# arpg/Kangaroo

Measured on AMD Instinct MI355X. Metric: kinectfusion_frames_per_sec_640x480_to_512cubed_tsdf, higher is better.
Workload: dtype f32

## Files before the change

include/kfx_debug.h:

```cpp
#ifndef KFX_DEBUG_H
#define KFX_DEBUG_H

#include "kfx.h"

#ifdef __cplusplus
extern "C" {
#endif

int kfx_debug_rmw(const kfx_volume* vol, int variant, kfx_stream stream);

int kfx_debug_div_uniform_check(float b, unsigned long long* d_out, kfx_stream stream);

int kfx_debug_div_core_check(unsigned seed, int per_divisor, unsigned long long* d_out, kfx_stream stream);
int kfx_debug_sqrt_core_check(unsigned long long* d_out, kfx_stream stream);
int kfx_debug_wave_xor_check(unsigned seed, unsigned long long* d_out, kfx_stream stream);

int kfx_debug_summary_export(kfx_sdf_summary* s, float tol, float vref, int fine_shift, void* R_out, void* C_out, int dims_out[12],
                             kfx_stream stream);


#ifdef __cplusplus
}
#endif
#endif
```

kangaroo_amd/csrc/debug.hip:

```cpp
#include "kfx_device.h"
#include "sampling.h"
#include "../../include/kfx_debug.h"

namespace kfx {

__global__ __launch_bounds__(256) void k_rmw_linear(float4* __restrict__ base, size_t n4)
{
    const size_t stride = (size_t)gridDim.x * blockDim.x;
    for (size_t i = (size_t)blockIdx.x * blockDim.x + threadIdx.x; i < n4; i += stride) {
        float4 c = base[i];
        c.y += 1.0f;
        c.w += 1.0f;
        base[i] = c;
    }
}

template <int ZC>
__global__ __launch_bounds__(256) void k_rmw_brick(unsigned char* vptr, size_t pitch, size_t img_pitch, int X, int Y, int Z)
{
    const int tid = threadIdx.x, lane = tid & 63, wv = tid >> 6;
    const int x0 = (blockIdx.x * 32 + (lane & 31)) * 2;
    const int y = blockIdx.y * 8 + wv * 2 + (lane >> 5);
    const int zbeg = blockIdx.z * ZC, zend = min(zbeg + ZC, Z);
    if (x0 >= X || y >= Y) return;
// ... 221 lines not shown
    default: return set_error(KFX_E_RANGE, "kfx_debug_rmw: variant");
    }
    return check_launch("kfx_debug_rmw");
}

extern "C" int kfx_debug_summary_export(kfx_sdf_summary* s, float tol, float vref, int fine_shift, void* R_out, void* C_out, int dims_out[12],
                                        kfx_stream stream)
{
    if (!s || !dims_out) return set_error(KFX_E_NULL, "kfx_debug_summary_export: null argument");
    if (fine_shift < 3 || fine_shift > 5) return set_error(KFX_E_RANGE, "kfx_debug_summary_export: fine_shift in [3, 5]");
    ClassView cv;
    summary_class_layout(s, fine_shift, cv);
    dims_out[0] = s->nbx; dims_out[1] = s->nby; dims_out[2] = s->nbz;
    dims_out[3] = cv.fine.first; dims_out[4] = cv.fine.rw; dims_out[5] = cv.fine.ny;
    dims_out[6] = cv.coarse.first; dims_out[7] = cv.coarse.rw; dims_out[8] = cv.coarse.ny;
    dims_out[9] = cv.words; dims_out[10] = s->n_coarse; dims_out[11] = (s->h_skippable && s->builds) ? ((volatile int*)s->h_skippable)[(s->builds - 1) % KFX_SUMMARY_RING] : -2;
    const size_t n = (size_t)s->nbx * s->nby * s->nbz;
    hipStream_t st = (hipStream_t)stream;
    if (R_out && hipMemcpyAsync(R_out, s->R, n * sizeof(float4), hipMemcpyDeviceToDevice, st) != hipSuccess) return set_error(KFX_E_RANGE, "kfx_debug_summary_export: copy");
    if (C_out) {
        if (int e = summary_classes_prepare(s, tol, vref, fine_shift, st)) return e;
        if (hipMemcpyAsync(C_out, s->C, (size_t)cv.words * sizeof(unsigned), hipMemcpyDeviceToDevice, st) != hipSuccess || hipStreamSynchronize(st) != hipSuccess)
            return set_error(KFX_E_RANGE, "kfx_debug_summary_export: copy");
        dims_out[11] = (s->h_skippable && s->builds) ? ((volatile int*)s->h_skippable)[(s->builds - 1) % KFX_SUMMARY_RING] : -2;
    }
    return 0;
}
```

kangaroo_amd/csrc/frame.hip:

```cpp
#include <cmath>
#include <cstdlib>
#include <new>

#include "kfx_device.h"

struct kfx_frame {
    kfx_frame_config cfg;
    kfx_sdf_summary* summary;
    int track;
    long long frames;
    int slots;
    hipEvent_t* ev;
    long long* ev_frame;
    unsigned char* ev_mask;
    unsigned mask;
    kfx_image texels;
};

using namespace kfx;

static int valid_image(const kfx_image& im, size_t elem)
{
    return im.ptr && im.w > 0 && im.h > 0 && im.pitch >= im.w * elem;
}
// ... 135 lines not shown
        f->ev_frame[(int)(f->frames % f->slots)] = -1;
    }
    const hipStream_t s = (hipStream_t)stream;
    int e = 0;
    const auto record = [&](int k) {
        if (!(m & (1u << k))) return;
        const hipError_t he = hipEventRecord(ev[k], s);
        if (he != hipSuccess) {
            (void)hipGetLastError();
            f->ev_mask[(int)(f->frames % f->slots)] &= (unsigned char)~(1u << k);
            if (!e) e = set_error((int)he, "kfx_frame_step: hipEventRecord");
        }
    };
    record(0);
    const kfx_image* tex = ((parts & KFX_FRAME_PREPROCESS) && (parts & KFX_FRAME_FUSE) && f->texels.ptr) ? &f->texels : nullptr;
    if (!e && (parts & KFX_FRAME_PREPROCESS)) {
        e = kfx_bilateral_f32(&c.filtered, src, c.bilateral_gs, c.bilateral_gr, c.bilateral_size, c.bilateral_minval, 1, stream);
        if (!e) e = depth_to_vbo_normals_texels(&c.vbo, &c.normals, &c.filtered, c.K, 1.0f, tex, stream);
    }
    record(1);
    if (!e && (parts & KFX_FRAME_FUSE))
        e = sdf_fuse_texels(&c.vol, f->track ? f->summary : nullptr, &c.filtered, &c.normals, tex, T_cw, c.K, c.trunc_dist, c.max_w, c.mincostheta, c.fuse_flags, stream);
    record(2);
    if (!e && (parts & KFX_FRAME_RAYCAST)) {
        if (f->track) e = kfx_raycast_sdf_tracked(&c.ray_depth, &c.ray_norm, &c.ray_img, &c.vol, f->summary, T_wc, c.K, c.near, c.far, c.trunc_dist, 1, stream);
        else e = kfx_raycast_sdf(&c.ray_depth, &c.ray_norm, &c.ray_img, &c.vol, T_wc, c.K, c.near, c.far, c.trunc_dist, 1, stream);
    }
    record(3);
    f->frames += 1;
    return e;
}

extern "C" int kfx_frame_timings(kfx_frame* f, long long first_frame, int n_frames, float* ms)
{
// ... 50 lines not shown
```

kangaroo_amd/csrc/kfx_device.h:

```cpp
#pragma once

#include <hip/hip_runtime.h>
#include <stddef.h>
#include <stdint.h>

#include "../../include/kfx.h"
#include "../../include/kfx_extras.h"

namespace kfx {

struct V3 { float x, y, z; };

__device__ __forceinline__ V3 v3(float x, float y, float z) { return V3{x, y, z}; }
__device__ __forceinline__ V3 operator+(V3 a, V3 b) { return V3{a.x + b.x, a.y + b.y, a.z + b.z}; }
__device__ __forceinline__ V3 operator-(V3 a, V3 b) { return V3{a.x - b.x, a.y - b.y, a.z - b.z}; }
__device__ __forceinline__ V3 operator*(V3 a, float s) { return V3{a.x * s, a.y * s, a.z * s}; }
__device__ __forceinline__ V3 div_cw(V3 a, V3 b) { return V3{a.x / b.x, a.y / b.y, a.z / b.z}; }
__device__ __forceinline__ V3 div_s(V3 a, float s) { const float inv = 1.0f / s; return a * inv; }
__device__ __forceinline__ float dot(V3 a, V3 b) { return a.x * b.x + a.y * b.y + a.z * b.z; }
__device__ __forceinline__ float length(V3 a) { return sqrtf(dot(a, a)); }
__device__ __forceinline__ float lerp(float a, float b, float t) { return a + t * (b - a); }
__device__ __forceinline__ V3 lerp(V3 a, V3 b, float t) { return a + (b - a) * t; }
__device__ __forceinline__ float clampf(float f, float a, float b) { return fmaxf(a, fminf(f, b)); }

// ... 111 lines not shown
}

#define KFX_SUMMARY_RING 8
struct kfx_sdf_summary {
    float4* R;
    int nbx, nby, nbz;
    int w, h, d;
    const unsigned char* base;
    size_t pitch, img_pitch;
    unsigned* C;
    int c_dirty;
    float c_tol, c_vref;
    int c_shift;
    int n_coarse;
    int* d_count;
    int* h_skippable;
    int* d_skippable;
    hipEvent_t build_done[8];
    unsigned builds;
    unsigned plain_calls;
    unsigned sweeps;
};
namespace kfx {
struct ClassLevel {
    int shift;
    int ny;
    int rw;
    int first;
};
struct ClassView {
    const unsigned* C;
    ClassLevel fine, coarse;
    int words;
    float vref;
    float tol;
    int amb_ok;
    int ox, oy, oz;
    float eps;
    int nx5, nz5, top_n, lds_words;
};
inline __host__ __device__ void class_level_up(const int nx, const int ny, const int nz, const int shift, const int first, ClassLevel& L, int& ux, int& uz, int& words)
{
    ux = (nx + 1) >> 1; uz = (nz + 1) >> 1;
    L.shift = shift; L.ny = (ny + 1) >> 1; L.rw = 2 * ((ux + 31) >> 5); L.first = first;
    words = (L.rw * L.ny * uz + 3) & ~3;
}
int summary_classes_prepare(kfx_sdf_summary* s, float tol, float vref, int fine_shift, hipStream_t stream);
void summary_class_layout(const kfx_sdf_summary* s, int fine_shift, ClassView& cv);
int summary_view_offset(const kfx_sdf_summary* s, const kfx_volume* view, int* ox, int* oy, int* oz);
}

namespace kfx {
int set_error(int code, const char* what);
int check_launch(const char* what);
int math_mode();
size_t texel_image_bytes(size_t w, size_t h);
int depth_to_vbo_normals_texels(const kfx_image* vbo, const kfx_image* nrm, const kfx_image* depth, const float K[4], float scale,
                                const kfx_image* texels, kfx_stream stream);
int sdf_fuse_slab_texels(const kfx_volume* vol, const kfx_slab* slab, const kfx_image* depth, const kfx_image* norm, const kfx_image* texels,
                         const float T_cw[12], const float K[4], float trunc_dist, float max_w, float mincostheta, unsigned flags, kfx_stream stream);
int sdf_fuse_texels(const kfx_volume* vol, kfx_sdf_summary* summary, const kfx_image* depth, const kfx_image* norm, const kfx_image* texels,
                    const float T_cw[12], const float K[4], float trunc_dist, float max_w, float mincostheta, unsigned flags, kfx_stream stream);
}
```

kangaroo_amd/csrc/preprocess.hip:

```cpp
#include <cstdlib>

#include "kfx_device.h"

namespace kfx {

constexpr int BIL_MAX_R = 16;

struct BilParams {
    const unsigned char* in;
    size_t in_pitch;
    unsigned char* out;
    size_t out_pitch;
    int w, h;
    int iw, ih;
    int R;
    float gs, gr;
    float minval;
    int use_minval;
};

template <typename Ti>
__device__ __forceinline__ float load_clamped(const BilParams& p, int x, int y)
{
    x = min(max(x, 0), p.iw - 1);
// ... 44 lines not shown
                    if (!p.use_minval || q >= p.minval) {
                        const float id = pc - q;
                        const float id2 = id * id;
                        const float iw = __expf(-(id2) / inv2gr);
                        const float w = srow[c] * iw;
                        sumw += w;
                        sum += w * q;
                    }
                }
            }
        }
        reinterpret_cast<float*>(p.out + (size_t)y * p.out_pitch)[x] = sum / sumw;
    }
}

template <typename Ti, int R>
__global__ __launch_bounds__(256) void k_bilateral_fast(const BilParams p)
{
    constexpr int TX = 16, TY = 16, D = 2 * R + 1, TW = TX + 2 * R, TH = TY + 2 * R;
    __shared__ float tile[TH * TW];
    __shared__ float sw[D * D];
    const int tid = threadIdx.x;
    const int bx = blockIdx.x * TX, by = blockIdx.y * TY;
    for (int i = tid; i < TW * TH; i += 256) {
        const int ty = i / TW, tx = i - ty * TW;
        tile[i] = load_clamped<Ti>(p, bx + tx - R, by + ty - R);
    }
    if (tid < D * D) {
        const int r = tid / D - R, c = tid % D - R;
        sw[tid] = __expf(-((float)(r * r + c * c)) / (2 * p.gs * p.gs));
    }
    __syncthreads();
    const int lx = tid % TX, ly = tid / TX;
    const int x = bx + lx, y = by + ly;
    if (x >= p.w || y >= p.h) return;
    const float k = -1.0f / (2 * p.gr * p.gr);
    const float pc = tile[(ly + R) * TW + lx + R];
    const bool check = p.use_minval != 0;
    float sum = 0.f, sumw = 0.f;
#pragma unroll
    for (int r = 0; r < D; ++r)
#pragma unroll
        for (int c = 0; c < D; ++c) {
            const float q = tile[(ly + r) * TW + lx + c];
            const bool ok = !check || q >= p.minval;
            const float id = pc - q;
            const float w = sw[r * D + c] * __expf(id * id * k);
            sumw += ok ? w : 0.f;
            sum += ok ? w * q : 0.f;
        }
    if (check && !(pc >= p.minval)) sum = sumw = 0.f;
    reinterpret_cast<float*>(p.out + (size_t)y * p.out_pitch)[x] = sum / sumw;
}

template <typename Ti>
__global__ __launch_bounds__(256) void k_bilateral_global(const BilParams p)
{
    const int x = blockIdx.x * 64 + (threadIdx.x & 63), y = blockIdx.y * 4 + (threadIdx.x >> 6);
    if (x >= p.w || y >= p.h) return;
    const float pc = (float)reinterpret_cast<const Ti*>(p.in + (size_t)y * p.in_pitch)[x];
    float sum = 0.f, sumw = 0.f;
    if (!p.use_minval || pc >= p.minval) {
        for (int r = -p.R; r <= p.R; ++r)
            for (int c = -p.R; c <= p.R; ++c) {
                const float q = load_clamped<Ti>(p, x + c, y + r);
                if (!p.use_minval || q >= p.minval) {
                    const float sd2 = (float)(r * r + c * c);
// ... 89 lines not shown
}

struct VboNrmParams {
    const unsigned char* in;
    size_t in_pitch;
    unsigned char *vbo, *nrm;
    size_t vpitch, npitch;
    int w, h;
    Intr K;
    float scale;
    unsigned char* tex;
    size_t tpitch;
    float* bmax;
    unsigned bw8;
};
__device__ __forceinline__ float4 vertex_of(const VboNrmParams& p, int u, int v)
{
    const float kz = p.scale * reinterpret_cast<const float*>(p.in + (size_t)v * p.in_pitch)[u];
    return make_float4(kz * ((float)u - p.K.u0) / p.K.fu, kz * ((float)v - p.K.v0) / p.K.fv, kz, 1.0f);
}
__global__ __launch_bounds__(256) void k_vbo_normals_f32(const VboNrmParams p)
{
    __shared__ float s_max[4][8];
    const int lane = threadIdx.x & 63, wv = threadIdx.x >> 6;
    const int u = blockIdx.x * 64 + lane, v = blockIdx.y * 4 + wv;
    float d = -__builtin_inff();
    if (u < p.w && v < p.h) {
        const float4 Vc = vertex_of(p, u, v);
        reinterpret_cast<float4*>(p.vbo + (size_t)v * p.vpitch)[u] = Vc;
        float4 N = make_float4(0.f, 0.f, 0.f, 0.f);
        if (u + 1 < p.w && v + 1 < p.h) {
            const float4 Vr = vertex_of(p, u + 1, v), Vu = vertex_of(p, u, v + 1);
            const V3 a = v3(Vr.x - Vc.x, Vr.y - Vc.y, Vr.z - Vc.z);
            const V3 b = v3(Vu.x - Vc.x, Vu.y - Vc.y, Vu.z - Vc.z);
            const V3 axb = v3(a.y * b.z - a.z * b.y, a.z * b.x - a.x * b.z, a.x * b.y - a.y * b.x);
            const float mag = length(axb);
            N = make_float4(-axb.x / mag, -axb.y / mag, -axb.z / mag, 1.0f);
        }
        reinterpret_cast<float4*>(p.nrm + (size_t)v * p.npitch)[u] = N;
        if (p.tex) {
            d = reinterpret_cast<const float*>(p.in + (size_t)v * p.in_pitch)[u];
            reinterpret_cast<float4*>(p.tex + (size_t)v * p.tpitch)[u] = make_float4(N.x, N.y, N.z, d);
        }
    }
    if (p.tex) {
        d = wave8_combine(fmaxf(d, -__builtin_inff()), [](float a, float b) { return fmaxf(a, b); });
        if ((lane & 7) == 0) s_max[wv][lane >> 3] = d;
        __syncthreads();
        if (threadIdx.x < 8)
            p.bmax[(size_t)blockIdx.y * p.bw8 + blockIdx.x * 8 + threadIdx.x] =
                fmaxf(fmaxf(s_max[0][threadIdx.x], s_max[1][threadIdx.x]), fmaxf(s_max[2][threadIdx.x], s_max[3][threadIdx.x]));
    }
}

struct EwParams {
    const unsigned char* in;
    size_t in_pitch;
    unsigned char* out;
    size_t out_pitch;
    int w, h;
    float s, offset;
};

__global__ __launch_bounds__(256) void k_scale_bias_f32(const EwParams p)
{
    const int x = blockIdx.x * 64 + (threadIdx.x & 63), y = blockIdx.y * 4 + (threadIdx.x >> 6);
// ... 407 lines not shown
    if (int e = check_image(depth, 4, "DepthToVbo+Normals: depth image")) return e;
    if (!K) return set_error(KFX_E_NULL, "DepthToVbo+Normals: null intrinsics");
    if (vbo->w == 0 || vbo->h == 0) return 0;
    if (nrm->w != vbo->w || nrm->h != vbo->h || depth->w < vbo->w || depth->h < vbo->h)
        return set_error(KFX_E_SHAPE, "DepthToVbo+Normals: image sizes");
    const size_t tpitch = (vbo->w * 16 + 255) / 256 * 256;
    if (texels && (!texels->ptr || texels->w != vbo->w || texels->h != vbo->h || texels->pitch != tpitch || ((uintptr_t)texels->ptr & 15)))
        return set_error(KFX_E_SHAPE, "DepthToVbo+Normals: texel image");
    VboNrmParams p{(const unsigned char*)depth->ptr, depth->pitch, (unsigned char*)vbo->ptr, (unsigned char*)nrm->ptr, vbo->pitch, nrm->pitch,
                   (int)vbo->w, (int)vbo->h, Intr{K[0], K[1], K[2], K[3]}, scale, texels ? (unsigned char*)texels->ptr : nullptr, texels ? tpitch : 0,
                   texels ? reinterpret_cast<float*>((unsigned char*)texels->ptr + tpitch * vbo->h) : nullptr, (unsigned)((vbo->w + 63) / 64 * 8)};
    hipLaunchKernelGGL(k_vbo_normals_f32, dim3(ceil_div(p.w, 64), ceil_div(p.h, 4)), dim3(256), 0, (hipStream_t)stream, p);
    return check_launch("kfx_depth_to_vbo_normals_f32");
}

struct PyrParams {
    const unsigned char* d0;
    size_t d0_pitch;
    unsigned char* d[4];
    size_t dpitch[4];
    unsigned char *vbo[4], *nrm[4];
    size_t vpitch[4], npitch[4];
    int w[4], h[4];
    Intr K[4];
    int levels;
    float scale;
};
__device__ __forceinline__ float4 pyr_vertex(const Intr& K, float scale, float depth, int u, int v)
{
    const float kz = scale * depth;
// ... 139 lines not shown
```

kangaroo_amd/csrc/raycast.hip:

```cpp
#include <cmath>
#include <cstdlib>

#include <hip/hip_fp16.h>

#include "kfx_device.h"
#include "sampling.h"

namespace kfx {

struct RayParams {
    VolView vol;
    V3 size;
    V3 dims1;
    V3 hi2;
    V3 voxel;
    V3 inv_size;
    int fastdiv, off32;
    Pose T;
    Intr K;
    unsigned char *dptr, *nptr, *iptr;
    size_t dpitch, npitch, ipitch;
    int w, h;
    float near, far, trunc;
    int subpix;
// ... 737 lines not shown
    static const int kb_env = [] { const char* e = getenv("KFX_RAYCAST_CLASS_KB"); const int v = e ? atoi(e) : 16; return v < 1 ? 1 : (v > 60 ? 60 : v); }();
    int fine = 3;
    for (; fine < 5; ++fine) {
        summary_class_layout(summary, fine, cl);
        if ((size_t)cl.words * 4 <= (size_t)kb_env * 1024) break;
    }
    summary_class_layout(summary, fine, cl);
    if ((size_t)cl.words * 4 > 60 * 1024) return 0;
    const float tol = math_mode() == KFX_MATH_FAST ? 1e-5f : 0.f;
    static const int force_env = [] { const char* e = getenv("KFX_RAYCAST_SUMMARY"); return e ? atoi(e) : 0; }();
    if (force_env < 0) return 0;
    const bool steer = force_env == 0 && summary->h_skippable;
    if (steer && summary->plain_calls && (summary->plain_calls++ % 8u) != 0u) return 0;
    if (int e = summary_classes_prepare(summary, tol, p.trunc, fine, (hipStream_t)stream)) return e;
    if (steer && summary->builds >= 3) {
        const unsigned ref = (summary->builds - 3) % KFX_SUMMARY_RING;
        (void)hipEventSynchronize(summary->build_done[ref]);
        const int known = ((volatile int*)summary->h_skippable)[ref];
        if (known >= 0 && (long long)known * 4 < summary->n_coarse) {
            if (!summary->plain_calls) summary->plain_calls = 1;
            return 0;
        }
        summary->plain_calls = 0;
    }
    cl.C = summary->C;
    cl.vref = p.trunc;
    cl.amb_ok = p.trunc >= p.voxel.x ? 1 : 0;
    cl.tol = tol;
    const double u24 = 1.0 / 16777216.0;
    double eps = 0.0;
    const float bmin[3] = {p.vol.bmin.x, p.vol.bmin.y, p.vol.bmin.z}, bmax[3] = {p.vol.bmax.x, p.vol.bmax.y, p.vol.bmax.z};
    const float size[3] = {p.size.x, p.size.y, p.size.z}, dims1[3] = {p.dims1.x, p.dims1.y, p.dims1.z};
    const float cw[3] = {p.T.m[3], p.T.m[7], p.T.m[11]};
// ... 336 lines not shown
```

kangaroo_amd/csrc/summary.hip:

```cpp
#include <algorithm>
#include <new>

#include "kfx_device.h"

namespace kfx {

__global__ __launch_bounds__(256) void k_summary_fill(float4* __restrict__ R, size_t n, float lo, float hi, int state)
{
    const size_t i = (size_t)blockIdx.x * 256 + threadIdx.x;
    if (i < n) R[i] = make_float4(lo, hi, __int_as_float(state), 0.f);
}

struct ClassBuild {
    const float4* R;
    unsigned* C;
    int nbx, nby, nbz;
    int shift, nx, ny, nz, rw;
    float lo_ok, hi_ok;
    const unsigned* src;
    int src_shift, src_nx, src_ny, src_nz, src_rw;
};
template <int M>
__device__ __forceinline__ int class_row(const ClassBuild& b, const long long wave)
{
    const float4* __restrict__ R = b.R;
    unsigned* __restrict__ C = b.C;
    const unsigned* __restrict__ src = b.src;
    const int nbx = b.nbx, nby = b.nby, nbz = b.nbz, shift = b.shift, nx = b.nx, ny = b.ny, rw = b.rw;
    const int src_shift = b.src_shift, src_nx = b.src_nx, src_ny = b.src_ny, src_nz = b.src_nz, src_rw = b.src_rw;
    const float lo_ok = b.lo_ok, hi_ok = b.hi_ok;
    const int lane = threadIdx.x & 63;
    const int chunks = (nx + 63) >> 6;
    const int chunk = (int)(wave % chunks), by = (int)((wave / chunks) % ny), bz = (int)(wave / ((long long)chunks * ny));
    const int bx = chunk * 64 + lane;
    int cls = 0;
    if (bx < nx) {
        bool all_nan = true, all_free = true, all_either = true;
        if constexpr (M == 0) {
            const int m = 1 << (shift - src_shift);
            for (int z0 = 0; z0 < m; z0 += 2) {
                uint2 w2[2][4];
#pragma unroll
                for (int dz = 0; dz < 2; ++dz)
#pragma unroll
                    for (int dy = 0; dy < 4; ++dy) {
                        const int z = min(bz * m + z0 + dz, src_nz - 1), y = min(by * m + min(dy, m - 1), src_ny - 1);
                        w2[dz][dy] = *reinterpret_cast<const uint2*>(src + ((size_t)z * src_ny + y) * src_rw + (((bx * m) >> 5) << 1));
                    }
// ... 29 lines not shown
#pragma unroll
                    for (int dx = 0; dx <= M; ++dx)
                        r[(dz * (M + 1) + dy) * (M + 1) + dx] =
                            R[((size_t)min(bz * M + dz, nbz - 1) * nby + min(by * M + dy, nby - 1)) * nbx + min(bx * M + dx, nbx - 1)];
#pragma unroll
            for (int k = 0; k < (M + 1) * (M + 1) * (M + 1); ++k) {
                const int st = __float_as_int(r[k].z);
                const bool in_band = r[k].x >= lo_ok && r[k].y <= hi_ok;
                all_nan = all_nan && st == 1;
                all_free = all_free && st == 0 && in_band;
                all_either = all_either && (st == 1 || in_band);
            }
        }
        cls = all_free ? 1 : (all_nan ? 2 : (all_either ? 3 : 0));
    }
    const unsigned long long p0 = __ballot(cls & 1), p1 = __ballot(cls & 2);
    if (lane == 0) {
        unsigned* row = C + ((size_t)bz * ny + by) * rw + chunk * 4;
        row[0] = (unsigned)p0; row[1] = (unsigned)p1;
        if (chunk * 4 + 2 < rw) { row[2] = (unsigned)(p0 >> 32); row[3] = (unsigned)(p1 >> 32); }
    }
    return __popcll(p0 | p1);
}

template <int M>
__global__ __launch_bounds__(256) void k_summary_classes(const ClassBuild b, const long long n_waves)
{
    const long long wave = (long long)blockIdx.x * 4 + (threadIdx.x >> 6);
    if (wave < n_waves) class_row<M>(b, wave);
}

template <int M>
__global__ __launch_bounds__(256) void k_summary_classes_coarse(const ClassBuild b, const long long n_waves, int* __restrict__ count, int* __restrict__ publish)
{
    __shared__ int s_count[4];
    const int wv = threadIdx.x >> 6;
    const long long wave = (long long)blockIdx.x * 4 + wv;
    const int n = wave < n_waves ? class_row<M>(b, wave) : 0;
    if ((threadIdx.x & 63) == 0) s_count[wv] = n;
    __syncthreads();
    if (threadIdx.x == 0) {
        atomicAdd(&count[0], s_count[0] + s_count[1] + s_count[2] + s_count[3]);
        __threadfence();
        if (atomicAdd(&count[1], 1) == (int)gridDim.x - 1) {
            __threadfence();
            const int total = atomicExch(&count[0], 0);
            count[1] = 0;
            __hip_atomic_store(publish, total, __ATOMIC_RELAXED, __HIP_MEMORY_SCOPE_SYSTEM);
        }
    }
}

__global__ __launch_bounds__(256) void k_summary_rebuild(float4* __restrict__ R, const unsigned char* __restrict__ base, size_t pitch, size_t img_pitch,
                                                         int w, int h, int d, int nbx, int nby, int nbz, int aligned16)
{
    const long long brick = (long long)blockIdx.x * 4 + (threadIdx.x >> 6);
    if (brick >= (long long)nbx * nby * nbz) return;
    const int lane = threadIdx.x & 63;
    const int bx = (int)(brick % nbx), by = (int)((brick / nbx) % nby), bz = (int)(brick / ((long long)nbx * nby));
    const int y = by * 8 + (lane & 7), z = bz * 8 + (lane >> 3), x0 = bx * 8;
    float lo = __builtin_inff(), hi = -__builtin_inff();
    bool nan = false, val = false;
    if (y < h && z < d) {
        const unsigned char* row = base + (size_t)z * img_pitch + (size_t)y * pitch + (size_t)x0 * 8;
// ... 43 lines not shown

void summary_class_layout(const kfx_sdf_summary* s, int fine_shift, ClassView& cv)
{
    class_level(cv.fine, fine_shift, s->w, s->h, 0);
    const int fw = fine_shift < 5 ? class_level_words(cv.fine, s->d) : 0;
    class_level(cv.coarse, 5, s->w, s->h, (fw + 3) & ~3);
    cv.words = cv.coarse.first + ((class_level_words(cv.coarse, s->d) + 3) & ~3);
}

int summary_classes_prepare(kfx_sdf_summary* s, float tol, float vref, int fine_shift, hipStream_t stream)
{
    if (!s->c_dirty && s->c_tol == tol && s->c_vref == vref && s->c_shift == fine_shift) return 0;
    ClassView cv;
    summary_class_layout(s, fine_shift, cv);
    const float lo_ok = vref - tol * vref, hi_ok = vref + tol * vref;
    for (int pass = 0; pass < 2; ++pass) {
        const ClassLevel& L = pass ? cv.coarse : cv.fine;
        if (!pass && fine_shift >= 5) continue;
        ClassBuild b;
        b.R = s->R; b.C = s->C + L.first;
        b.nbx = s->nbx; b.nby = s->nby; b.nbz = s->nbz;
        b.shift = L.shift; b.nx = ceil_div(s->w, 1 << L.shift); b.ny = L.ny; b.nz = ceil_div(s->d, 1 << L.shift); b.rw = L.rw;
        b.lo_ok = lo_ok; b.hi_ok = hi_ok;
        const bool from_fine = pass && fine_shift < 5;
        b.src = from_fine ? s->C + cv.fine.first : nullptr;
        b.src_shift = cv.fine.shift; b.src_nx = ceil_div(s->w, 1 << cv.fine.shift); b.src_ny = cv.fine.ny;
        b.src_nz = ceil_div(s->d, 1 << cv.fine.shift); b.src_rw = cv.fine.rw;
        const long long waves = (long long)ceil_div(b.nx, 64) * b.ny * b.nz;
        if (pass) {
            const dim3 grid((unsigned)((waves + 3) / 4));
            const unsigned slot = s->builds % KFX_SUMMARY_RING;
            int* publish = s->d_skippable + (s->h_skippable ? slot : 0);
            if (from_fine) hipLaunchKernelGGL(k_summary_classes_coarse<0>, grid, dim3(256), 0, stream, b, waves, s->d_count, publish);
            else hipLaunchKernelGGL(k_summary_classes_coarse<4>, grid, dim3(256), 0, stream, b, waves, s->d_count, publish);
            if (s->h_skippable) (void)hipEventRecord(s->build_done[slot], stream);
            s->builds += 1;
        } else if (L.shift == 3) {
            hipLaunchKernelGGL(k_summary_classes<1>, dim3((unsigned)((waves + 3) / 4)), dim3(256), 0, stream, b, waves);
        } else {
            hipLaunchKernelGGL(k_summary_classes<2>, dim3((unsigned)((waves + 3) / 4)), dim3(256), 0, stream, b, waves);
        }
        if (int e = check_launch("kfx_sdf_summary (classes)")) return e;
    }
    s->c_dirty = 0; s->c_tol = tol; s->c_vref = vref; s->c_shift = fine_shift;
    return 0;
}

int summary_view_offset(const kfx_sdf_summary* s, const kfx_volume* view, int* ox, int* oy, int* oz)
{
    if (!s || !view || !view->ptr) return set_error(KFX_E_NULL, "summary: null argument");
    if (view->pitch != s->pitch || view->img_pitch != s->img_pitch) return set_error(KFX_E_SHAPE, "summary: the volume is not a view of the summary's volume (pitches)");
    const unsigned char* q = static_cast<const unsigned char*>(view->ptr);
    if (q < s->base) return set_error(KFX_E_SHAPE, "summary: the volume is not a view of the summary's volume");
    const size_t off = (size_t)(q - s->base);
    const size_t z = off / s->img_pitch, rem = off % s->img_pitch, y = rem / s->pitch, xb = rem % s->pitch;
    if (xb % 8 || z + view->d > (size_t)s->d || y + view->h > (size_t)s->h || xb / 8 + view->w > (size_t)s->w)
        return set_error(KFX_E_SHAPE, "summary: the volume is not a view of the summary's volume (extent)");
    *ox = (int)(xb / 8); *oy = (int)y; *oz = (int)z;
// ... 5 lines not shown
using namespace kfx;

extern "C" int kfx_sdf_summary_create(kfx_sdf_summary** out, const kfx_volume* vol)
{
    if (!out || !vol || !vol->ptr) return set_error(KFX_E_NULL, "kfx_sdf_summary_create: null argument");
    if (vol->w < 2 || vol->h < 2 || vol->d < 2 || vol->w > 65535 || vol->h > 65535 || vol->d > 65535) return set_error(KFX_E_SHAPE, "kfx_sdf_summary_create: volume dimensions");
    kfx_sdf_summary* s = new (std::nothrow) kfx_sdf_summary;
    if (!s) return set_error(KFX_E_RANGE, "kfx_sdf_summary_create: out of memory");
    s->nbx = ceil_div((int)vol->w, 8); s->nby = ceil_div((int)vol->h, 8); s->nbz = ceil_div((int)vol->d, 8);
    s->w = (int)vol->w; s->h = (int)vol->h; s->d = (int)vol->d;
    s->base = static_cast<const unsigned char*>(vol->ptr);
    s->pitch = vol->pitch; s->img_pitch = vol->img_pitch;
    s->R = nullptr; s->C = nullptr; s->d_count = nullptr; s->h_skippable = nullptr; s->d_skippable = nullptr;
    s->c_dirty = 1; s->c_tol = -1.f; s->c_vref = 0.f; s->c_shift = 0; s->sweeps = 0;
    s->builds = 0; s->plain_calls = 0;
    for (auto& e : s->build_done) e = nullptr;
    s->n_coarse = ceil_div(s->w, 32) * ceil_div(s->h, 32) * ceil_div(s->d, 32);
    const size_t n = (size_t)s->nbx * s->nby * s->nbz;
    ClassView cv;
    summary_class_layout(s, 3, cv);
    bool ok = hipMalloc((void**)&s->R, n * sizeof(float4)) == hipSuccess && hipMalloc((void**)&s->C, (size_t)cv.words * sizeof(unsigned)) == hipSuccess &&
              hipMalloc((void**)&s->d_count, 2 * sizeof(int)) == hipSuccess && hipMemset(s->d_count, 0, 2 * sizeof(int)) == hipSuccess;
    if (ok && hipHostMalloc((void**)&s->h_skippable, KFX_SUMMARY_RING * sizeof(int), hipHostMallocMapped) == hipSuccess) {
        for (int i = 0; i < KFX_SUMMARY_RING; ++i) s->h_skippable[i] = -1;
        bool evs = hipHostGetDevicePointer((void**)&s->d_skippable, s->h_skippable, 0) == hipSuccess;
        for (int i = 0; evs && i < KFX_SUMMARY_RING; ++i) evs = hipEventCreateWithFlags(&s->build_done[i], hipEventDisableTiming) == hipSuccess;
        if (!evs) {
            for (auto& e : s->build_done) { if (e) (void)hipEventDestroy(e); e = nullptr; }
            (void)hipHostFree(s->h_skippable);
            s->h_skippable = nullptr;
        }
    } else {
        s->h_skippable = nullptr;
    }
    if (ok && !s->h_skippable) {
        (void)hipGetLastError();
        ok = hipMalloc((void**)&s->d_skippable, sizeof(int)) == hipSuccess;
    }
    if (!ok) {
        (void)hipGetLastError();
        kfx_sdf_summary_destroy(s);
        return set_error(KFX_E_NODEVICE, "kfx_sdf_summary_create: hipMalloc");
    }
    *out = s;
    return kfx_sdf_summary_invalidate(s, nullptr);
}

extern "C" int kfx_sdf_summary_destroy(kfx_sdf_summary* s)
{
    if (!s) return 0;
    (void)hipDeviceSynchronize();
    if (s->R) (void)hipFree(s->R);
    if (s->C) (void)hipFree(s->C);
    if (s->d_count) (void)hipFree(s->d_count);
    for (auto& e : s->build_done) if (e) (void)hipEventDestroy(e);
    if (s->h_skippable) (void)hipHostFree(s->h_skippable);
    else if (s->d_skippable) (void)hipFree(s->d_skippable);
    delete s;
    return 0;
}

extern "C" int kfx_sdf_summary_rebuild(kfx_sdf_summary* s, kfx_stream stream)
{
    if (!s) return set_error(KFX_E_NULL, "kfx_sdf_summary_rebuild: null summary");
    const long long n = (long long)s->nbx * s->nby * s->nbz;
    const int aligned16 = ((((uintptr_t)s->base) | s->pitch | s->img_pitch) & 15) == 0;
    hipLaunchKernelGGL(k_summary_rebuild, dim3((unsigned)((n + 3) / 4)), dim3(256), 0, (hipStream_t)stream, s->R, s->base, s->pitch, s->img_pitch,
                       s->w, s->h, s->d, s->nbx, s->nby, s->nbz, aligned16);
    s->c_dirty = 1;
    return check_launch("kfx_sdf_summary_rebuild");
// ... 27 lines not shown
```

Baseline: 2409.

## Fuse bilateral filter with vertex/normal/texel pass and streamline summary class publishing

Adds a fused preprocessing kernel that runs the bilateral filter into shared memory, including a one-pixel halo, and computes vertices, normals, texels and block depth maxima in the same launch. This removes one kernel launch and the global-memory round trip of the filtered depth. The summary class build also gets a single fused kernel for the 16-voxel fine level. Skippable-count publishing switches from event records to a sequence-tagged 64-bit word, which avoids per-build hipEventRecord calls. The cost is redundant halo bilateral work, 320-thread blocks and more complex publication logic.

```diff
diff --git a/include/kfx_debug.h b/include/kfx_debug.h
--- a/include/kfx_debug.h
+++ b/include/kfx_debug.h
@@ -18,6 +18,9 @@
 int kfx_debug_summary_export(kfx_sdf_summary* s, float tol, float vref, int fine_shift, void* R_out, void* C_out, int dims_out[12],
                              kfx_stream stream);
 
+int kfx_debug_preprocess(const kfx_image* filtered, const kfx_image* vbo, const kfx_image* nrm, const kfx_image* raw, float gs, float gr,
+                         unsigned size, float minval, int use_minval, const float K[4], void* texels, int fused, kfx_stream stream);
+size_t kfx_debug_texel_image_bytes(size_t w, size_t h);
 
 #ifdef __cplusplus
 }
diff --git a/kangaroo_amd/csrc/debug.hip b/kangaroo_amd/csrc/debug.hip
--- a/kangaroo_amd/csrc/debug.hip
+++ b/kangaroo_amd/csrc/debug.hip
@@ -259,7 +259,7 @@
     dims_out[0] = s->nbx; dims_out[1] = s->nby; dims_out[2] = s->nbz;
     dims_out[3] = cv.fine.first; dims_out[4] = cv.fine.rw; dims_out[5] = cv.fine.ny;
     dims_out[6] = cv.coarse.first; dims_out[7] = cv.coarse.rw; dims_out[8] = cv.coarse.ny;
-    dims_out[9] = cv.words; dims_out[10] = s->n_coarse; dims_out[11] = (s->h_skippable && s->builds) ? ((volatile int*)s->h_skippable)[(s->builds - 1) % KFX_SUMMARY_RING] : -2;
+    dims_out[9] = cv.words; dims_out[10] = s->n_coarse; dims_out[11] = (s->h_skippable && s->builds) ? summary_published(s, s->builds - 1) : -2;
     const size_t n = (size_t)s->nbx * s->nby * s->nbz;
     hipStream_t st = (hipStream_t)stream;
     if (R_out && hipMemcpyAsync(R_out, s->R, n * sizeof(float4), hipMemcpyDeviceToDevice, st) != hipSuccess) return set_error(KFX_E_RANGE, "kfx_debug_summary_export: copy");
@@ -267,7 +267,19 @@
         if (int e = summary_classes_prepare(s, tol, vref, fine_shift, st)) return e;
         if (hipMemcpyAsync(C_out, s->C, (size_t)cv.words * sizeof(unsigned), hipMemcpyDeviceToDevice, st) != hipSuccess || hipStreamSynchronize(st) != hipSuccess)
             return set_error(KFX_E_RANGE, "kfx_debug_summary_export: copy");
-        dims_out[11] = (s->h_skippable && s->builds) ? ((volatile int*)s->h_skippable)[(s->builds - 1) % KFX_SUMMARY_RING] : -2;
+        dims_out[11] = (s->h_skippable && s->builds) ? summary_published(s, s->builds - 1) : -2;
     }
     return 0;
 }
+
+extern "C" int kfx_debug_preprocess(const kfx_image* filtered, const kfx_image* vbo, const kfx_image* nrm, const kfx_image* raw, float gs, float gr,
+                                    unsigned size, float minval, int use_minval, const float K[4], void* texels, int fused, kfx_stream stream)
+{
+    if (!vbo) return set_error(KFX_E_NULL, "kfx_debug_preprocess: null argument");
+    const kfx_image tex{(vbo->w * 16 + 255) / 256 * 256, texels, vbo->w, vbo->h};
+    if (fused) return preprocess_frame(filtered, vbo, nrm, raw, gs, gr, size, minval, use_minval, K, 1.0f, texels ? &tex : nullptr, stream);
+    if (int e = kfx_bilateral_f32(filtered, raw, gs, gr, size, minval, use_minval, stream)) return e;
+    return depth_to_vbo_normals_texels(vbo, nrm, filtered, K, 1.0f, texels ? &tex : nullptr, stream);
+}
+
+extern "C" size_t kfx_debug_texel_image_bytes(size_t w, size_t h) { return texel_image_bytes(w, h); }
diff --git a/kangaroo_amd/csrc/frame.hip b/kangaroo_amd/csrc/frame.hip
--- a/kangaroo_amd/csrc/frame.hip
+++ b/kangaroo_amd/csrc/frame.hip
@@ -173,10 +173,8 @@
     };
     record(0);
     const kfx_image* tex = ((parts & KFX_FRAME_PREPROCESS) && (parts & KFX_FRAME_FUSE) && f->texels.ptr) ? &f->texels : nullptr;
-    if (!e && (parts & KFX_FRAME_PREPROCESS)) {
-        e = kfx_bilateral_f32(&c.filtered, src, c.bilateral_gs, c.bilateral_gr, c.bilateral_size, c.bilateral_minval, 1, stream);
-        if (!e) e = depth_to_vbo_normals_texels(&c.vbo, &c.normals, &c.filtered, c.K, 1.0f, tex, stream);
-    }
+    if (!e && (parts & KFX_FRAME_PREPROCESS))
+        e = preprocess_frame(&c.filtered, &c.vbo, &c.normals, src, c.bilateral_gs, c.bilateral_gr, c.bilateral_size, c.bilateral_minval, 1, c.K, 1.0f, tex, stream);
     record(1);
     if (!e && (parts & KFX_FRAME_FUSE))
         e = sdf_fuse_texels(&c.vol, f->track ? f->summary : nullptr, &c.filtered, &c.normals, tex, T_cw, c.K, c.trunc_dist, c.max_w, c.mincostheta, c.fuse_flags, stream);
diff --git a/kangaroo_amd/csrc/kfx_device.h b/kangaroo_amd/csrc/kfx_device.h
--- a/kangaroo_amd/csrc/kfx_device.h
+++ b/kangaroo_amd/csrc/kfx_device.h
@@ -149,9 +149,9 @@
     int c_shift;
     int n_coarse;
     int* d_count;
-    int* h_skippable;
-    int* d_skippable;
-    hipEvent_t build_done[8];
+    unsigned long long* h_skippable;
+    unsigned long long* d_skippable;
+    hipStream_t build_stream[KFX_SUMMARY_RING];
     unsigned builds;
     unsigned plain_calls;
     unsigned sweeps;
@@ -181,6 +181,11 @@
     words = (L.rw * L.ny * uz + 3) & ~3;
 }
 int summary_classes_prepare(kfx_sdf_summary* s, float tol, float vref, int fine_shift, hipStream_t stream);
+inline int summary_published(const kfx_sdf_summary* s, unsigned b)
+{
+    const unsigned long long w = reinterpret_cast<volatile const unsigned long long*>(s->h_skippable)[b % KFX_SUMMARY_RING];
+    return (unsigned)(w >> 32) == b + 1u ? (int)(unsigned)w : -1;
+}
 void summary_class_layout(const kfx_sdf_summary* s, int fine_shift, ClassView& cv);
 int summary_view_offset(const kfx_sdf_summary* s, const kfx_volume* view, int* ox, int* oy, int* oz);
 }
@@ -192,6 +197,8 @@
 size_t texel_image_bytes(size_t w, size_t h);
 int depth_to_vbo_normals_texels(const kfx_image* vbo, const kfx_image* nrm, const kfx_image* depth, const float K[4], float scale,
                                 const kfx_image* texels, kfx_stream stream);
+int preprocess_frame(const kfx_image* filtered, const kfx_image* vbo, const kfx_image* nrm, const kfx_image* raw, float gs, float gr,
+                     unsigned size, float minval, int use_minval, const float K[4], float scale, const kfx_image* texels, kfx_stream stream);
 int sdf_fuse_slab_texels(const kfx_volume* vol, const kfx_slab* slab, const kfx_image* depth, const kfx_image* norm, const kfx_image* texels,
                          const float T_cw[12], const float K[4], float trunc_dist, float max_w, float mincostheta, unsigned flags, kfx_stream stream);
 int sdf_fuse_texels(const kfx_volume* vol, kfx_sdf_summary* summary, const kfx_image* depth, const kfx_image* norm, const kfx_image* texels,
diff --git a/kangaroo_amd/csrc/preprocess.hip b/kangaroo_amd/csrc/preprocess.hip
--- a/kangaroo_amd/csrc/preprocess.hip
+++ b/kangaroo_amd/csrc/preprocess.hip
@@ -82,26 +82,19 @@
     }
 }
 
-template <typename Ti, int R>
-__global__ __launch_bounds__(256) void k_bilateral_fast(const BilParams p)
-{
-    constexpr int TX = 16, TY = 16, D = 2 * R + 1, TW = TX + 2 * R, TH = TY + 2 * R;
-    __shared__ float tile[TH * TW];
-    __shared__ float sw[D * D];
-    const int tid = threadIdx.x;
-    const int bx = blockIdx.x * TX, by = blockIdx.y * TY;
-    for (int i = tid; i < TW * TH; i += 256) {
-        const int ty = i / TW, tx = i - ty * TW;
-        tile[i] = load_clamped<Ti>(p, bx + tx - R, by + ty - R);
-    }
-    if (tid < D * D) {
-        const int r = tid / D - R, c = tid % D - R;
-        sw[tid] = __expf(-((float)(r * r + c * c)) / (2 * p.gs * p.gs));
-    }
-    __syncthreads();
-    const int lx = tid % TX, ly = tid / TX;
-    const int x = bx + lx, y = by + ly;
-    if (x >= p.w || y >= p.h) return;
+template <int R>
+__device__ __forceinline__ void bilateral_fast_weights(float* sw, const BilParams& p)
+{
+    constexpr int D = 2 * R + 1;
+    if (threadIdx.x < D * D) {
+        const int r = threadIdx.x / D - R, c = threadIdx.x % D - R;
+        sw[threadIdx.x] = __expf(-((float)(r * r + c * c)) / (2 * p.gs * p.gs));
+    }
+}
+template <int R, int TW>
+__device__ __forceinline__ float bilateral_fast_pixel(const float* tile, const float* sw, const BilParams& p, int lx, int ly)
+{
+    constexpr int D = 2 * R + 1;
     const float k = -1.0f / (2 * p.gr * p.gr);
     const float pc = tile[(ly + R) * TW + lx + R];
     const bool check = p.use_minval != 0;
@@ -118,7 +111,26 @@
             sum += ok ? w * q : 0.f;
         }
     if (check && !(pc >= p.minval)) sum = sumw = 0.f;
-    reinterpret_cast<float*>(p.out + (size_t)y * p.out_pitch)[x] = sum / sumw;
+    return sum / sumw;
+}
+template <typename Ti, int R>
+__global__ __launch_bounds__(256) void k_bilateral_fast(const BilParams p)
+{
+    constexpr int TX = 16, TY = 16, D = 2 * R + 1, TW = TX + 2 * R, TH = TY + 2 * R;
+    __shared__ float tile[TH * TW];
+    __shared__ float sw[D * D];
+    const int tid = threadIdx.x;
+    const int bx = blockIdx.x * TX, by = blockIdx.y * TY;
+    for (int i = tid; i < TW * TH; i += 256) {
+        const int ty = i / TW, tx = i - ty * TW;
+        tile[i] = load_clamped<Ti>(p, bx + tx - R, by + ty - R);
+    }
+    bilateral_fast_weights<R>(sw, p);
+    __syncthreads();
+    const int lx = tid % TX, ly = tid / TX;
+    const int x = bx + lx, y = by + ly;
+    if (x >= p.w || y >= p.h) return;
+    reinterpret_cast<float*>(p.out + (size_t)y * p.out_pitch)[x] = bilateral_fast_pixel<R, TW>(tile, sw, p, lx, ly);
 }
 
 template <typename Ti>
@@ -238,10 +250,22 @@
     float* bmax;
     unsigned bw8;
 };
+__device__ __forceinline__ float4 vertex_at(const VboNrmParams& p, float z, int u, int v)
+{
+    const float kz = p.scale * z;
+    return make_float4(kz * ((float)u - p.K.u0) / p.K.fu, kz * ((float)v - p.K.v0) / p.K.fv, kz, 1.0f);
+}
+__device__ __forceinline__ float4 normal_of(const float4 Vc, const float4 Vr, const float4 Vu)
+{
+    const V3 a = v3(Vr.x - Vc.x, Vr.y - Vc.y, Vr.z - Vc.z);
+    const V3 b = v3(Vu.x - Vc.x, Vu.y - Vc.y, Vu.z - Vc.z);
+    const V3 axb = v3(a.y * b.z - a.z * b.y, a.z * b.x - a.x * b.z, a.x * b.y - a.y * b.x);
+    const float mag = length(axb);
+    return make_float4(-axb.x / mag, -axb.y / mag, -axb.z / mag, 1.0f);
+}
 __device__ __forceinline__ float4 vertex_of(const VboNrmParams& p, int u, int v)
 {
-    const float kz = p.scale * reinterpret_cast<const float*>(p.in + (size_t)v * p.in_pitch)[u];
-    return make_float4(kz * ((float)u - p.K.u0) / p.K.fu, kz * ((float)v - p.K.v0) / p.K.fv, kz, 1.0f);
+    return vertex_at(p, reinterpret_cast<const float*>(p.in + (size_t)v * p.in_pitch)[u], u, v);
 }
 __global__ __launch_bounds__(256) void k_vbo_normals_f32(const VboNrmParams p)
 {
@@ -253,14 +277,7 @@
         const float4 Vc = vertex_of(p, u, v);
         reinterpret_cast<float4*>(p.vbo + (size_t)v * p.vpitch)[u] = Vc;
         float4 N = make_float4(0.f, 0.f, 0.f, 0.f);
-        if (u + 1 < p.w && v + 1 < p.h) {
-            const float4 Vr = vertex_of(p, u + 1, v), Vu = vertex_of(p, u, v + 1);
-            const V3 a = v3(Vr.x - Vc.x, Vr.y - Vc.y, Vr.z - Vc.z);
-            const V3 b = v3(Vu.x - Vc.x, Vu.y - Vc.y, Vu.z - Vc.z);
-            const V3 axb = v3(a.y * b.z - a.z * b.y, a.z * b.x - a.x * b.z, a.x * b.y - a.y * b.x);
-            const float mag = length(axb);
-            N = make_float4(-axb.x / mag, -axb.y / mag, -axb.z / mag, 1.0f);
-        }
+        if (u + 1 < p.w && v + 1 < p.h) N = normal_of(Vc, vertex_of(p, u + 1, v), vertex_of(p, u, v + 1));
         reinterpret_cast<float4*>(p.nrm + (size_t)v * p.npitch)[u] = N;
         if (p.tex) {
             d = reinterpret_cast<const float*>(p.in + (size_t)v * p.in_pitch)[u];
@@ -274,6 +291,63 @@
         if (threadIdx.x < 8)
             p.bmax[(size_t)blockIdx.y * p.bw8 + blockIdx.x * 8 + threadIdx.x] =
                 fmaxf(fmaxf(s_max[0][threadIdx.x], s_max[1][threadIdx.x]), fmaxf(s_max[2][threadIdx.x], s_max[3][threadIdx.x]));
+    }
+}
+
+struct PreParams {
+    BilParams b;
+    VboNrmParams v;
+    unsigned bh4;
+};
+template <int R>
+__global__ __launch_bounds__(320) void k_preprocess_fast(const PreParams q)
+{
+    constexpr int D = 2 * R + 1, FW = 17, TW = FW + 2 * R;
+    __shared__ float tile[TW * TW];
+    __shared__ float sw[D * D];
+    __shared__ float ft[FW * FW];
+    const BilParams& p = q.b;
+    const VboNrmParams& pv = q.v;
+    const int tid = threadIdx.x;
+    const int bx = blockIdx.x * 16, by = blockIdx.y * 16;
+    for (int i = tid; i < TW * TW; i += 320) {
+        const int ty = i / TW, tx = i - ty * TW;
+        tile[i] = load_clamped<float>(p, bx + tx - R, by + ty - R);
+    }
+    bilateral_fast_weights<R>(sw, p);
+    __syncthreads();
+    const int lx = tid & 15, ly = tid >> 4;
+    const int u = bx + lx, v = by + ly;
+    const bool in = u < p.w && v < p.h;
+    if (tid < 256) {
+        const float f = bilateral_fast_pixel<R, TW>(tile, sw, p, lx, ly);
+        ft[ly * FW + lx] = f;
+        if (in) reinterpret_cast<float*>(p.out + (size_t)v * p.out_pitch)[u] = f;
+    } else if (tid < 256 + 2 * FW - 1) {
+        const int t = tid - 256, hx = t < 16 ? 16 : t - 16, hy = t < 16 ? t : 16;
+        ft[hy * FW + hx] = bilateral_fast_pixel<R, TW>(tile, sw, p, hx, hy);
+    }
+    __syncthreads();
+    if (tid >= 256) return;
+    float d = -__builtin_inff();
+    if (in) {
+        const float z = ft[ly * FW + lx];
+        const float4 Vc = vertex_at(pv, z, u, v);
+        reinterpret_cast<float4*>(pv.vbo + (size_t)v * pv.vpitch)[u] = Vc;
+        float4 N = make_float4(0.f, 0.f, 0.f, 0.f);
+        if (u + 1 < pv.w && v + 1 < pv.h) N = normal_of(Vc, vertex_at(pv, ft[ly * FW + lx + 1], u + 1, v), vertex_at(pv, ft[(ly + 1) * FW + lx], u, v + 1));
+        reinterpret_cast<float4*>(pv.nrm + (size_t)v * pv.npitch)[u] = N;
+        if (pv.tex) {
+            d = z;
+            reinterpret_cast<float4*>(pv.tex + (size_t)v * pv.tpitch)[u] = make_float4(N.x, N.y, N.z, d);
+        }
+    }
+    if (pv.tex) {
+        d = wave8_combine(fmaxf(d, -__builtin_inff()), [](float a, float b) { return fmaxf(a, b); });
+        d = fmaxf(d, __shfl_xor(d, 16, 64));
+        d = fmaxf(d, __shfl_xor(d, 32, 64));
+        const int lane = tid & 63, by4 = blockIdx.y * 4 + (tid >> 6);
+        if ((lane == 0 || lane == 8) && by4 < (int)q.bh4) pv.bmax[(size_t)by4 * pv.bw8 + blockIdx.x * 2 + (lane >> 3)] = d;
     }
 }
 
@@ -711,6 +785,43 @@
     return check_launch("kfx_depth_to_vbo_normals_f32");
 }
 
+int kfx::preprocess_frame(const kfx_image* filtered, const kfx_image* vbo, const kfx_image* nrm, const kfx_image* raw, float gs, float gr,
+                          unsigned size, float minval, int use_minval, const float K[4], float scale, const kfx_image* texels, kfx_stream stream)
+{
+    if (math_mode() != KFX_MATH_FAST || size < 1 || size > 3) {
+        if (int e = kfx_bilateral_f32(filtered, raw, gs, gr, size, minval, use_minval, stream)) return e;
+        return depth_to_vbo_normals_texels(vbo, nrm, filtered, K, scale, texels, stream);
+    }
+    if (int e = check_image(filtered, 4, "BilateralFilter: output image")) return e;
+    if (int e = check_image(raw, 4, "BilateralFilter: input image")) return e;
+    if (filtered->w == 0 || filtered->h == 0) return 0;
+    if (raw->w == 0 || raw->h == 0) return set_error(KFX_E_SHAPE, "BilateralFilter: empty input");
+    if (raw->w < filtered->w || raw->h < filtered->h) return set_error(KFX_E_SHAPE, "BilateralFilter: input smaller than output");
+    if (int e = check_image(vbo, 16, "DepthToVbo+Normals: vbo image")) return e;
+    if (int e = check_image(nrm, 16, "DepthToVbo+Normals: normal image")) return e;
+    if (!K) return set_error(KFX_E_NULL, "DepthToVbo+Normals: null intrinsics");
+    if (vbo->w != filtered->w || vbo->h != filtered->h || nrm->w != vbo->w || nrm->h != vbo->h)
+        return set_error(KFX_E_SHAPE, "DepthToVbo+Normals: image sizes");
+    const size_t tpitch = (vbo->w * 16 + 255) / 256 * 256;
+    if (texels && (!texels->ptr || texels->w != vbo->w || texels->h != vbo->h || texels->pitch != tpitch || ((uintptr_t)texels->ptr & 15)))
+        return set_error(KFX_E_SHAPE, "DepthToVbo+Normals: texel image");
+    PreParams q;
+    q.b.in = (const unsigned char*)raw->ptr; q.b.in_pitch = raw->pitch;
+    q.b.out = (unsigned char*)filtered->ptr; q.b.out_pitch = filtered->pitch;
+    q.b.w = (int)filtered->w; q.b.h = (int)filtered->h; q.b.iw = (int)raw->w; q.b.ih = (int)raw->h;
+    q.b.R = (int)size; q.b.gs = gs; q.b.gr = gr; q.b.minval = minval; q.b.use_minval = use_minval ? 1 : 0;
+    q.v = VboNrmParams{nullptr, 0, (unsigned char*)vbo->ptr, (unsigned char*)nrm->ptr, vbo->pitch, nrm->pitch,
+                       (int)vbo->w, (int)vbo->h, Intr{K[0], K[1], K[2], K[3]}, scale, texels ? (unsigned char*)texels->ptr : nullptr, texels ? tpitch : 0,
+                       texels ? reinterpret_cast<float*>((unsigned char*)texels->ptr + tpitch * vbo->h) : nullptr, (unsigned)((vbo->w + 63) / 64 * 8)};
+    q.bh4 = (unsigned)((vbo->h + 3) / 4);
+    const dim3 grid(ceil_div(q.b.w, 64) * 4, ceil_div(q.b.h, 16));
+    const hipStream_t s = (hipStream_t)stream;
+    if (size == 3) hipLaunchKernelGGL(k_preprocess_fast<3>, grid, dim3(320), 0, s, q);
+    else if (size == 2) hipLaunchKernelGGL(k_preprocess_fast<2>, grid, dim3(320), 0, s, q);
+    else hipLaunchKernelGGL(k_preprocess_fast<1>, grid, dim3(320), 0, s, q);
+    return check_launch("kfx_frame (preprocess)");
+}
+
 struct PyrParams {
     const unsigned char* d0;
     size_t d0_pitch;
diff --git a/kangaroo_amd/csrc/raycast.hip b/kangaroo_amd/csrc/raycast.hip
--- a/kangaroo_amd/csrc/raycast.hip
+++ b/kangaroo_amd/csrc/raycast.hip
@@ -775,9 +775,16 @@
     if (steer && summary->plain_calls && (summary->plain_calls++ % 8u) != 0u) return 0;
     if (int e = summary_classes_prepare(summary, tol, p.trunc, fine, (hipStream_t)stream)) return e;
     if (steer && summary->builds >= 3) {
-        const unsigned ref = (summary->builds - 3) % KFX_SUMMARY_RING;
-        (void)hipEventSynchronize(summary->build_done[ref]);
-        const int known = ((volatile int*)summary->h_skippable)[ref];
+        const unsigned ref = summary->builds - 3;
+        int known = summary_published(summary, ref);
+        for (unsigned spin = 1; known < 0; ++spin) {
+            if (!(spin & 1023u) && hipStreamQuery(summary->build_stream[ref % KFX_SUMMARY_RING]) != hipErrorNotReady) {
+                (void)hipGetLastError();
+                known = summary_published(summary, ref);
+                break;
+            }
+            known = summary_published(summary, ref);
+        }
         if (known >= 0 && (long long)known * 4 < summary->n_coarse) {
             if (!summary->plain_calls) summary->plain_calls = 1;
             return 0;
diff --git a/kangaroo_amd/csrc/summary.hip b/kangaroo_amd/csrc/summary.hip
--- a/kangaroo_amd/csrc/summary.hip
+++ b/kangaroo_amd/csrc/summary.hip
@@ -21,17 +21,14 @@
     int src_shift, src_nx, src_ny, src_nz, src_rw;
 };
 template <int M>
-__device__ __forceinline__ int class_row(const ClassBuild& b, const long long wave)
+__device__ __forceinline__ int class_entry(const ClassBuild& b, const int chunk, const int by, const int bz)
 {
     const float4* __restrict__ R = b.R;
-    unsigned* __restrict__ C = b.C;
     const unsigned* __restrict__ src = b.src;
-    const int nbx = b.nbx, nby = b.nby, nbz = b.nbz, shift = b.shift, nx = b.nx, ny = b.ny, rw = b.rw;
+    const int nbx = b.nbx, nby = b.nby, nbz = b.nbz, shift = b.shift, nx = b.nx;
     const int src_shift = b.src_shift, src_nx = b.src_nx, src_ny = b.src_ny, src_nz = b.src_nz, src_rw = b.src_rw;
     const float lo_ok = b.lo_ok, hi_ok = b.hi_ok;
     const int lane = threadIdx.x & 63;
-    const int chunks = (nx + 63) >> 6;
-    const int chunk = (int)(wave % chunks), by = (int)((wave / chunks) % ny), bz = (int)(wave / ((long long)chunks * ny));
     const int bx = chunk * 64 + lane;
     int cls = 0;
     if (bx < nx) {
@@ -91,13 +88,24 @@
         }
         cls = all_free ? 1 : (all_nan ? 2 : (all_either ? 3 : 0));
     }
+    return cls;
+}
+__device__ __forceinline__ int class_store(const ClassBuild& b, const int chunk, const int by, const int bz, const int cls)
+{
     const unsigned long long p0 = __ballot(cls & 1), p1 = __ballot(cls & 2);
-    if (lane == 0) {
-        unsigned* row = C + ((size_t)bz * ny + by) * rw + chunk * 4;
+    if ((threadIdx.x & 63) == 0) {
+        unsigned* row = b.C + ((size_t)bz * b.ny + by) * b.rw + chunk * 4;
         row[0] = (unsigned)p0; row[1] = (unsigned)p1;
-        if (chunk * 4 + 2 < rw) { row[2] = (unsigned)(p0 >> 32); row[3] = (unsigned)(p1 >> 32); }
+        if (chunk * 4 + 2 < b.rw) { row[2] = (unsigned)(p0 >> 32); row[3] = (unsigned)(p1 >> 32); }
     }
     return __popcll(p0 | p1);
+}
+template <int M>
+__device__ __forceinline__ int class_row(const ClassBuild& b, const long long wave)
+{
+    const int chunks = (b.nx + 63) >> 6;
+    const int chunk = (int)(wave % chunks), by = (int)((wave / chunks) % b.ny), bz = (int)(wave / ((long long)chunks * b.ny));
+    return class_store(b, chunk, by, bz, class_entry<M>(b, chunk, by, bz));
 }
 
 template <int M>
@@ -107,8 +115,21 @@
     if (wave < n_waves) class_row<M>(b, wave);
 }
 
+__device__ __forceinline__ void class_count_publish(const int n, int* __restrict__ count, unsigned long long* __restrict__ publish, const unsigned seq)
+{
+    atomicAdd(&count[0], n);
+    __threadfence();
+    if (atomicAdd(&count[1], 1) == (int)gridDim.x - 1) {
+        __threadfence();
+        const int total = atomicExch(&count[0], 0);
+        count[1] = 0;
+        __hip_atomic_store(publish, ((unsigned long long)seq << 32) | (unsigned)total, __ATOMIC_RELAXED, __HIP_MEMORY_SCOPE_SYSTEM);
+    }
+}
+
 template <int M>
-__global__ __launch_bounds__(256) void k_summary_classes_coarse(const ClassBuild b, const long long n_waves, int* __restrict__ count, int* __restrict__ publish)
+__global__ __launch_bounds__(256) void k_summary_classes_coarse(const ClassBuild b, const long long n_waves, int* __restrict__ count,
+                                                                unsigned long long* __restrict__ publish, const unsigned seq)
 {
     __shared__ int s_count[4];
     const int wv = threadIdx.x >> 6;
@@ -116,15 +137,44 @@
     const int n = wave < n_waves ? class_row<M>(b, wave) : 0;
     if ((threadIdx.x & 63) == 0) s_count[wv] = n;
     __syncthreads();
-    if (threadIdx.x == 0) {
-        atomicAdd(&count[0], s_count[0] + s_count[1] + s_count[2] + s_count[3]);
-        __threadfence();
-        if (atomicAdd(&count[1], 1) == (int)gridDim.x - 1) {
-            __threadfence();
-            const int total = atomicExch(&count[0], 0);
-            count[1] = 0;
-            __hip_atomic_store(publish, total, __ATOMIC_RELAXED, __HIP_MEMORY_SCOPE_SYSTEM);
-        }
+    if (threadIdx.x == 0) class_count_publish(s_count[0] + s_count[1] + s_count[2] + s_count[3], count, publish, seq);
+}
+
+__global__ __launch_bounds__(256) void k_summary_classes_16(const ClassBuild f, const ClassBuild c, int* __restrict__ count,
+                                                            unsigned long long* __restrict__ publish, const unsigned seq)
+{
+    __shared__ int s_cls[4][64];
+    const int wv = threadIdx.x >> 6, lane = threadIdx.x & 63;
+    const int chunks = (f.nx + 63) >> 6;
+    const int chunk = (int)(blockIdx.x % chunks), cy = (int)((blockIdx.x / chunks) % c.ny), cz = (int)(blockIdx.x / (chunks * c.ny));
+    const int fy = 2 * cy + (wv & 1), fz = 2 * cz + (wv >> 1);
+    if (fy < f.ny && fz < f.nz) {
+        const int cls = class_entry<2>(f, chunk, fy, fz);
+        class_store(f, chunk, fy, fz, cls);
+        s_cls[wv][lane] = cls;
+    }
+    __syncthreads();
+    if (wv) return;
+    const int cx = chunk * 32 + lane;
+    int cls = 0;
+    if (lane < 32 && cx < c.nx) {
+        bool all_nan = true, all_free = true, all_either = true;
+        for (int dz = 0; dz < 2; ++dz)
+            for (int dy = 0; dy < 2; ++dy)
+                for (int dx = 0; dx < 2; ++dx) {
+                    const int z = min(2 * cz + dz, f.nz - 1) - 2 * cz, y = min(2 * cy + dy, f.ny - 1) - 2 * cy, x = min(2 * cx + dx, f.nx - 1) - chunk * 64;
+                    const int e = s_cls[z * 2 + y][x];
+                    all_free = all_free && e == 1;
+                    all_nan = all_nan && e == 2;
+                    all_either = all_either && e != 0;
+                }
+        cls = all_free ? 1 : (all_nan ? 2 : (all_either ? 3 : 0));
+    }
+    const unsigned long long p0 = __ballot(cls & 1), p1 = __ballot(cls & 2);
+    if (lane == 0) {
+        unsigned* row = c.C + ((size_t)cz * c.ny + cy) * c.rw + chunk * 2;
+        row[0] = (unsigned)p0; row[1] = (unsigned)p1;
+        class_count_publish(__popcll(p0 | p1), count, publish, seq);
     }
 }
 
@@ -198,10 +248,10 @@
     ClassView cv;
     summary_class_layout(s, fine_shift, cv);
     const float lo_ok = vref - tol * vref, hi_ok = vref + tol * vref;
+    ClassBuild lv[2];
     for (int pass = 0; pass < 2; ++pass) {
         const ClassLevel& L = pass ? cv.coarse : cv.fine;
-        if (!pass && fine_shift >= 5) continue;
-        ClassBuild b;
+        ClassBuild& b = lv[pass];
         b.R = s->R; b.C = s->C + L.first;
         b.nbx = s->nbx; b.nby = s->nby; b.nbz = s->nbz;
         b.shift = L.shift; b.nx = ceil_div(s->w, 1 << L.shift); b.ny = L.ny; b.nz = ceil_div(s->d, 1 << L.shift); b.rw = L.rw;
@@ -210,22 +260,26 @@
         b.src = from_fine ? s->C + cv.fine.first : nullptr;
         b.src_shift = cv.fine.shift; b.src_nx = ceil_div(s->w, 1 << cv.fine.shift); b.src_ny = cv.fine.ny;
         b.src_nz = ceil_div(s->d, 1 << cv.fine.shift); b.src_rw = cv.fine.rw;
-        const long long waves = (long long)ceil_div(b.nx, 64) * b.ny * b.nz;
-        if (pass) {
-            const dim3 grid((unsigned)((waves + 3) / 4));
-            const unsigned slot = s->builds % KFX_SUMMARY_RING;
-            int* publish = s->d_skippable + (s->h_skippable ? slot : 0);
-            if (from_fine) hipLaunchKernelGGL(k_summary_classes_coarse<0>, grid, dim3(256), 0, stream, b, waves, s->d_count, publish);
-            else hipLaunchKernelGGL(k_summary_classes_coarse<4>, grid, dim3(256), 0, stream, b, waves, s->d_count, publish);
-            if (s->h_skippable) (void)hipEventRecord(s->build_done[slot], stream);
-            s->builds += 1;
-        } else if (L.shift == 3) {
-            hipLaunchKernelGGL(k_summary_classes<1>, dim3((unsigned)((waves + 3) / 4)), dim3(256), 0, stream, b, waves);
+    }
+    const auto waves = [](const ClassBuild& b) { return (long long)ceil_div(b.nx, 64) * b.ny * b.nz; };
+    const auto wgs = [](long long w) { return dim3((unsigned)((w + 3) / 4)); };
+    const unsigned slot = s->builds % KFX_SUMMARY_RING, seq = s->builds + 1u;
+    unsigned long long* publish = s->d_skippable + (s->h_skippable ? slot : 0);
+    if (fine_shift == 4) {
+        const long long n = (long long)ceil_div(lv[0].nx, 64) * lv[1].ny * lv[1].nz;
+        hipLaunchKernelGGL(k_summary_classes_16, dim3((unsigned)n), dim3(256), 0, stream, lv[0], lv[1], s->d_count, publish, seq);
+    } else {
+        if (fine_shift == 3) {
+            hipLaunchKernelGGL(k_summary_classes<1>, wgs(waves(lv[0])), dim3(256), 0, stream, lv[0], waves(lv[0]));
+            if (int e = check_launch("kfx_sdf_summary (classes)")) return e;
+            hipLaunchKernelGGL(k_summary_classes_coarse<0>, wgs(waves(lv[1])), dim3(256), 0, stream, lv[1], waves(lv[1]), s->d_count, publish, seq);
         } else {
-            hipLaunchKernelGGL(k_summary_classes<2>, dim3((unsigned)((waves + 3) / 4)), dim3(256), 0, stream, b, waves);
+            hipLaunchKernelGGL(k_summary_classes_coarse<4>, wgs(waves(lv[1])), dim3(256), 0, stream, lv[1], waves(lv[1]), s->d_count, publish, seq);
         }
-        if (int e = check_launch("kfx_sdf_summary (classes)")) return e;
-    }
+    }
+    if (int e = check_launch("kfx_sdf_summary (classes)")) return e;
+    s->build_stream[slot] = stream;
+    s->builds += 1;
     s->c_dirty = 0; s->c_tol = tol; s->c_vref = vref; s->c_shift = fine_shift;
     return 0;
 }
@@ -261,19 +315,16 @@
     s->R = nullptr; s->C = nullptr; s->d_count = nullptr; s->h_skippable = nullptr; s->d_skippable = nullptr;
     s->c_dirty = 1; s->c_tol = -1.f; s->c_vref = 0.f; s->c_shift = 0; s->sweeps = 0;
     s->builds = 0; s->plain_calls = 0;
-    for (auto& e : s->build_done) e = nullptr;
+    for (auto& st : s->build_stream) st = nullptr;
     s->n_coarse = ceil_div(s->w, 32) * ceil_div(s->h, 32) * ceil_div(s->d, 32);
     const size_t n = (size_t)s->nbx * s->nby * s->nbz;
     ClassView cv;
     summary_class_layout(s, 3, cv);
     bool ok = hipMalloc((void**)&s->R, n * sizeof(float4)) == hipSuccess && hipMalloc((void**)&s->C, (size_t)cv.words * sizeof(unsigned)) == hipSuccess &&
               hipMalloc((void**)&s->d_count, 2 * sizeof(int)) == hipSuccess && hipMemset(s->d_count, 0, 2 * sizeof(int)) == hipSuccess;
-    if (ok && hipHostMalloc((void**)&s->h_skippable, KFX_SUMMARY_RING * sizeof(int), hipHostMallocMapped) == hipSuccess) {
-        for (int i = 0; i < KFX_SUMMARY_RING; ++i) s->h_skippable[i] = -1;
-        bool evs = hipHostGetDevicePointer((void**)&s->d_skippable, s->h_skippable, 0) == hipSuccess;
-        for (int i = 0; evs && i < KFX_SUMMARY_RING; ++i) evs = hipEventCreateWithFlags(&s->build_done[i], hipEventDisableTiming) == hipSuccess;
-        if (!evs) {
-            for (auto& e : s->build_done) { if (e) (void)hipEventDestroy(e); e = nullptr; }
+    if (ok && hipHostMalloc((void**)&s->h_skippable, KFX_SUMMARY_RING * sizeof(unsigned long long), hipHostMallocMapped) == hipSuccess) {
+        for (int i = 0; i < KFX_SUMMARY_RING; ++i) s->h_skippable[i] = 0;
+        if (hipHostGetDevicePointer((void**)&s->d_skippable, s->h_skippable, 0) != hipSuccess) {
             (void)hipHostFree(s->h_skippable);
             s->h_skippable = nullptr;
         }
@@ -282,7 +333,7 @@
     }
     if (ok && !s->h_skippable) {
         (void)hipGetLastError();
-        ok = hipMalloc((void**)&s->d_skippable, sizeof(int)) == hipSuccess;
+        ok = hipMalloc((void**)&s->d_skippable, sizeof(unsigned long long)) == hipSuccess;
     }
     if (!ok) {
         (void)hipGetLastError();
@@ -300,7 +351,6 @@
     if (s->R) (void)hipFree(s->R);
     if (s->C) (void)hipFree(s->C);
     if (s->d_count) (void)hipFree(s->d_count);
-    for (auto& e : s->build_done) if (e) (void)hipEventDestroy(e);
     if (s->h_skippable) (void)hipHostFree(s->h_skippable);
     else if (s->d_skippable) (void)hipFree(s->d_skippable);
     delete s;
```

New measurement: 2409, median of 6. About the same (+0.0%).
